# snap-research/3dgp

Hardware: AMD Instinct MI355X
Metric: generator-forward img/s @256^2, 64 steps (higher is better)
Workload: dtype f32; 1 GPU; BASELINE configs[2]: ImageNet 256x256, 64(+64) ray steps, cmax 512, c_dim 1000, tri-plane 512^2 x 96, full HIP path; batch_per_gpu=16, global_batch=16, img_resolution=256, num_ray_steps=64, depth_adaptor=False, parallelism=dp1 (batch-sharded, weights replicated)

## Files before the change

### 3dgp_amd/csrc/modconv.hip

```cpp
#include <type_traits>
#include "common.h"
#include <stdlib.h>

#ifndef TDGP_AB_NO_SCALAR_WV
#define TDGP_AB_NO_SCALAR_WV 0
#endif
#ifndef TDGP_AB_NO_PACKED_EPI
#define TDGP_AB_NO_PACKED_EPI 0
#endif
#ifndef TDGP_AB_FIR_SERIAL
#define TDGP_AB_FIR_SERIAL 0
#endif
#if TDGP_AB_NO_SCALAR_WV
#define TDGP_WAVE_INDEX(tid) ((tid) >> 6)
#else
#define TDGP_WAVE_INDEX(tid) __builtin_amdgcn_readfirstlane((tid) >> 6)
#endif

namespace {

typedef float f32x16 __attribute__((ext_vector_type(16)));

constexpr int KC3 = 4;

// ... 2741 lines not shown
                TDGP_LAUNCH("conv_mfma_kernel", conv3s_mfma_kernel, dim3((W >> 5) * cdiv(B * (H + 1), 8), cdiv(Cout, 64)), dim3(256), lds, s, q);
            } else if (g_conv_arith == 0 && TDGP_WINO4F_MAXCIN > 0 && out_layout == 0 && Cin <= TDGP_WINO4F_MAXCIN && (Cin & 15) == 0 && (Cout & 63) == 0 && wino4_txl(H, W) == 4 &&
                       wino4_shape_ok(B, Cin, Cout, H, W, k, up) && pi.wino4_floats > 0 && (int64_t)B * ((H * W) >> 9) * (Cout >> 6) >= 256 && !skip && ((uintptr_t)x & 15) == 0 &&
                       ((uintptr_t)y & 15) == 0 && (!noise || (((uintptr_t)noise & 15) == 0 && (noise_bstride & 3) == 0))) {
                float* vbuf = (float*)((char*)workspace + wl.wino_v);
                int* ticket = (int*)((char*)vbuf + ((wino4_v_bytes(wino4_sub_batch(B, Cin, Cout, H, W), Cin, H, W) + 255) / 256 * 256));
                const int cus = tdgp_cu_count(), nxcd = (cus % 8 == 0 && cus >= 64) ? 8 : 1, per = cus / nxcd, nsl = Cout >> 6;
                int rs = 1;
                while (rs * 2 <= nsl && (per % (rs * 2)) == 0 && (rs * 2) * 64 + per / (rs * 2) * 32 < rs * 64 + per / rs * 32) rs *= 2;
                Wino4fParams q;
                q.x = x; q.styles = styles; q.u = wp + pi.wp_floats + pi.wsq_floats + pi.wsplit_floats + pi.wbf_floats + pi.wino_floats; q.e = e;
                q.B = B; q.Cin = Cin; q.Cout = Cout; q.H = H; q.W = W; q.u_bytes = (uint32_t)(pi.wino4_floats * 4); q.x_bytes = c.x_bytes; q.st_bytes = c.st_bytes;
                q.nz_bytes = noise ? (uint32_t)(((noise_bstride ? (int64_t)(B - 1) * noise_bstride : 0) + (int64_t)H * W) * 4) : 0u;
                q.gxn = W / 64; q.gyn = H / 8; q.rs = rs; q.rt = per / rs; q.nxcd = nxcd; q.ticket = ticket;
                const size_t lds = (size_t)W4F_LDS_FLOATS * 4;
                TDGP_ONCE_PER_DEVICE((void)hipFuncSetAttribute((const void*)conv3_wino4f_kernel, hipFuncAttributeMaxDynamicSharedMemorySize, (int)lds););
                TDGP_CHECK(hipMemsetAsync(ticket, 0, 32, s) == hipSuccess, TDGP_ELAUNCH, "modconv2d: clearing the item counters failed");
                TDGP_LAUNCH("conv_wino4f_kernel", conv3_wino4f_kernel, dim3((unsigned)(nxcd * per)), dim3(512), lds, s, q);
            } else if (arith_wino4() && wino4_shape_ok(B, Cin, Cout, H, W, k, up, out_layout == 0) && pi.wino4_floats > 0 && (out_layout == 0 || out_layout == 2) && !skip && ((uintptr_t)x & 15) == 0 &&
                       ((uintptr_t)y & 15) == 0 && (!noise || (((uintptr_t)noise & 15) == 0 && (noise_bstride & 3) == 0))) {
                float* vbuf = (float*)((char*)workspace + wl.wino_v);
#ifndef TDGP_WINO4_PAIR
#define TDGP_WINO4_PAIR 1
#endif
                constexpr bool pairk = TDGP_WINO4_PAIR && W4_BM == 32;
                const int bpc = (W4_BM == 64 || pairk) ? 1 : 2;
                int ksl = (out_layout == 0 && !wino4_shape_ok(B, Cin, Cout, H, W, k, up)) ? wino4_ksplit_log2(B, Cin, Cout, H, W) : 0;
                const int64_t kslice = (int64_t)B * Cout * H * W;
                if ((kslice << ksl) > wl.partial_floats) ksl = 0;
                const int cus = tdgp_cu_count(), nxcd = (cus % 8 == 0 && cus >= 64) ? 8 : 1, per = cus / nxcd * bpc, nsl = cdiv(Cout, W4_BM) << ksl;
                int rs = 1;
                const int tpi = pairk ? 64 : 32;
                while (rs * 2 <= nsl && (per % (rs * 2)) == 0 && (rs * 2) * W4_BM + per / (rs * 2) * tpi < rs * W4_BM + per / rs * tpi) rs *= 2;
                const size_t lds = pairk ? (size_t)(8 * W4_UCH + 3 * W4_BM + 4) * 4 : (size_t)(2 * W4_STAGE + 2 * W4_BM + 4) * 4;
                TDGP_ONCE_PER_DEVICE((void)hipFuncSetAttribute((const void*)conv3_wino4_kernel<false, pairk>, hipFuncAttributeMaxDynamicSharedMemorySize, (int)lds); (void)hipFuncSetAttribute((const void*)conv3_wino4_kernel<true, pairk>, hipFuncAttributeMaxDynamicSharedMemorySize, (int)lds););
                const int bsub = ksl ? B : wino4_sub_batch(B, Cin, Cout, H, W);
                int* ticket = (int*)((char*)vbuf + ((wino4_v_bytes(wino4_sub_batch(B, Cin, Cout, H, W), Cin, H, W) + 255) / 256 * 256));
                for (int b0 = 0; b0 < B; b0 += bsub) {
                    const int bn = std::min(bsub, B - b0);
                    Wino4Params q;
                    q.v = vbuf; q.u = wp + pi.wp_floats + pi.wsq_floats + pi.wsplit_floats + pi.wbf_floats + pi.wino_floats; q.e = e;
                    q.e.y = y + (int64_t)b0 * Cout * H * W;
                    q.ups = out_layout == 2 ? 1 : 0;
                    if (e.dcoef) q.e.dcoef = e.dcoef + (int64_t)b0 * Cout;
                    if (e.noise) q.e.noise = e.noise + (int64_t)b0 * noise_bstride;
                    q.e.B = bn;
                    q.B = bn; q.Cin = Cin; q.Cout = Cout; q.CoutP = pi.CoutP; q.H = H; q.W = W;
                    q.v_bytes = (uint32_t)wino4_v_bytes(bn, Cin, H, W); q.u_bytes = (uint32_t)(pi.wino4_floats * 4);
                    q.txl = wino4_txl(H, W); q.gxn = W / (4 << q.txl); q.gyn = H / (128 >> q.txl);
                    q.rs = rs; q.rt = per / rs; q.nxcd = nxcd; q.ticket = ticket; q.ksl = ksl; q.partial = partial;
                    const int ntg = q.gxn * q.gyn * bn;
                    TDGP_LAUNCH("wino4_input_kernel", wino4_input_kernel, dim3((unsigned)(ntg * pi.nch4)), dim3(128), 0, s, x + (int64_t)b0 * Cin * H * W,
                                styles ? styles + (int64_t)b0 * Cin : nullptr, vbuf, bn, Cin, H, W, q.gxn, q.gyn, pi.nch4, q.txl, ticket);
                    if (q.ups) TDGP_LAUNCH("upconv_wino4_kernel", (conv3_wino4_kernel<true, pairk>), dim3((unsigned)(nxcd * per)), dim3(pairk ? 512 : W4_NW * 64), lds, s, q);
                    else TDGP_LAUNCH("conv_wino4_kernel", (conv3_wino4_kernel<false, pairk>), dim3((unsigned)(nxcd * per)), dim3(pairk ? 512 : W4_NW * 64), lds, s, q);
                    if (ksl) TDGP_LAUNCH("splitk_reduce_kernel", splitk_reduce_kernel, dim3((int)min((int64_t)2048, cdiv64(kslice, 256))), dim3(256), 0, s, partial, 1 << ksl, e);
                }
            } else if (k == 3 && (arith_wino4() || g_conv_arith == 3) && wino_ok(B, Cin, Cout, H, W) && out_layout == 0 && !skip && ((uintptr_t)x & 15) == 0 && ((uintptr_t)y & 7) == 0 &&
                       (!noise || (((uintptr_t)noise & 7) == 0 && (noise_bstride & 1) == 0))) {
                WinoParams q;
                q.x = x; q.u = wp + pi.wp_floats + pi.wsq_floats + pi.wsplit_floats + pi.wbf_floats; q.styles = styles; q.e = e;
                q.B = B; q.Cin = Cin; q.Cout = Cout; q.CoutP = pi.CoutP; q.H = H; q.W = W;
                q.x_bytes = c.x_bytes; q.u_bytes = (uint32_t)(pi.wino_floats * 4);
                const size_t lds = wino_lds_bytes(Cin);
                TDGP_ONCE_PER_DEVICE((void)hipFuncSetAttribute((const void*)conv3_wino_kernel, hipFuncAttributeMaxDynamicSharedMemorySize, 160 * 1024););
                if (TDGP_WINO_PERSIST) {
                    const int cus = tdgp_cu_count();
// ... 237 lines not shown
```

### 3dgp_amd/csrc/modconv_wino4.inc

```

typedef float f32x4 __attribute__((ext_vector_type(4)));

struct Wino4Params {
    const float* v; const float* u;
    EpiParams e;
    int B, Cin, Cout, CoutP, H, W;
    uint32_t v_bytes, u_bytes;
    int gxn, gyn;
    int txl;
    int rs, rt;
    int nxcd;
    int* ticket;
    int ups;
    int ksl;
    float* partial;
};

__device__ __forceinline__ void wino4_bt(const float (&d)[6], float (&t)[6]) {
    t[0] = fmaf_(1.5f, d[3] - d[1], fmaf_(-2.0f, d[2], d[0] + d[4]));
    t[1] = fmaf_(2.5f, d[3], fmaf_(0.5f, d[2], d[4] - d[1]));
    t[2] = fmaf_(-2.5f, d[2], fmaf_(0.5f, d[3], d[1] + d[4]));
    t[3] = fmaf_(2.0f, d[3] - d[1], d[4] - d[2]);
    t[4] = fmaf_(0.5f, d[1] - d[3], d[4] - d[2]);
    t[5] = fmaf_(1.5f, d[4] - d[2], fmaf_(-2.0f, d[3], d[1] + d[5]));
// ... 22 lines not shown
#pragma unroll
        for (int i = 0; i < 6; i++) col[i] = pr == 0 ? (w4_f2){acc[6 * i + j][0], acc[6 * i + j][1]} : (w4_f2){acc[6 * i + j][2], acc[6 * i + j][3]};
        w4_f2 y4[4];
        wino4_at2(col, y4);
#pragma unroll
        for (int a = 0; a < 4; a++) t[a][j] = y4[a];
    }
#pragma unroll
    for (int a = 0; a < 4; a++) wino4_at2(t[a], yy[a]);
}
template <int ACT>
__device__ __forceinline__ w4_f2 finish_pair(const EpiParams& e, w4_f2 v, w4_f2 d2, float nz, w4_f2 b2) {
    static_assert(ACT == 1 || ACT == 3, "packed output stage: linear / leaky ReLU without clamp");
    w4_f2 x = (v * d2 + (w4_f2){nz, nz}) + b2;
    if constexpr (ACT == 3) {
        const w4_f2 xa = x * (w4_f2){e.alpha, e.alpha};
        x = (w4_f2){__builtin_fmaxf(x.x, xa.x), __builtin_fmaxf(x.y, xa.y)};
    }
    return x * (w4_f2){e.gain, e.gain};
}

#ifndef TDGP_WINO4_MIN_C
#define TDGP_WINO4_MIN_C 64
#endif
#ifndef TDGP_WINO4_BM
#define TDGP_WINO4_BM 32
#endif
constexpr int W4_BM = TDGP_WINO4_BM, W4_NW = W4_BM / 8;
constexpr int W4_UCH = 9 * 4 * W4_BM * 4, W4_VCH = 9 * 4 * 32 * 4;
constexpr int W4_UP = W4_UCH / 256, W4_PAD = W4_BM == 64 ? 2 : 0;
constexpr int W4_NPW = (W4_UP + 18 + W4_PAD) / W4_NW;
constexpr int W4_STAGE = W4_UCH + W4_VCH + W4_PAD * 256;
static_assert((W4_UP + 18 + W4_PAD) % W4_NW == 0 && (W4_BM == 32 || W4_BM == 64), "wino4: piece count");

__global__ __launch_bounds__(256) void pack_wino4_kernel(const float* __restrict__ w, float* __restrict__ u, int Cout, int Cin, int nslice, int nch4) {
    const int64_t total = (int64_t)nslice * nch4 * W4_UCH;
    const double G[6][3] = {{1.0, 0.0, 0.0}, {1.0 / 3, 1.0 / 3, 1.0 / 3}, {-1.0 / 3, 1.0 / 3, -1.0 / 3}, {-16.0 / 15, -8.0 / 15, -4.0 / 15},
                            {1.0 / 15, -2.0 / 15, 4.0 / 15}, {0.0, 0.0, 1.0}};
    for (int64_t idx = blockIdx.x * (int64_t)blockDim.x + threadIdx.x; idx < total; idx += (int64_t)gridDim.x * blockDim.x) {
        const int e = (int)(idx & 3), cp = (int)(idx >> 2) % W4_BM, k = (int)((idx >> 2) / W4_BM) & 3;
        int64_t r = idx / (16 * W4_BM);
        const int xi4 = (int)(r % 9); r /= 9;
        const int ch = (int)(r % nch4), sl = (int)(r / nch4);
        const int o = sl * W4_BM + cp, c = ch * 4 + k, xi = 4 * xi4 + e, i = xi / 6, j = xi % 6;
        double v = 0.0;
        if (o < Cout && c < Cin) {
            const float* g = w + ((int64_t)o * Cin + c) * 9;
            for (int a = 0; a < 3; a++)
                for (int b = 0; b < 3; b++) v += G[i][a] * (double)g[a * 3 + b] * G[j][b];
        }
        u[idx] = (float)v;
    }
}

__global__ __launch_bounds__(128) void wino4_input_kernel(const float* __restrict__ x, const float* __restrict__ styles, float* __restrict__ v, int B, int Cin,
                                                          int H, int W, int gxn, int gyn, int nch4, int txl, int* __restrict__ ticket) {
    if (blockIdx.x == 0 && threadIdx.x < 8) ticket[threadIdx.x] = 0;
    const int k = threadIdx.x >> 5, t = threadIdx.x & 31, tx = t & ((1 << txl) - 1), ty = t >> txl;
    const int64_t blk = blockIdx.x;
    const int ch = (int)(blk % nch4);
    const int tg = (int)(blk / nch4);
    const int gx = tg % gxn, gy = (tg / gxn) % gyn, b = tg / (gxn * gyn);
    const int c = ch * 4 + k;
    const bool cok = c < Cin;
    const float s = (styles && cok) ? styles[b * Cin + c] : 1.0f;
    const int y0 = gy * (128 >> txl) + ty * 4 - 1, x0 = gx * (4 << txl) + tx * 4;
// ... 87 lines not shown
        const int q = wvx + 8 * i;
        dma(du, (uint32_t)__builtin_amdgcn_readfirstlane((int)(ust_lds + (uint32_t)q * 1024u)), lane16 + (uint32_t)q * 1024u, uo);
    };
    auto pairV = [&](int i, uint32_t vst_lds) {
        const int q = wvx + 8 * i;
        const bool second = i > 2 || (i == 2 && wvx >= 2);
        const int pc = second ? q - 18 : q;
        dma(dv, (uint32_t)__builtin_amdgcn_readfirstlane((int)(vst_lds + (second ? (uint32_t)(W4_VCH * 4) : 0u) + (uint32_t)pc * 1024u)), lane16 + (uint32_t)pc * 1024u, second ? vo1 : vo);
    };
    auto pair_offsets = [&](int cu, int cv) {
        uo = (uint32_t)__builtin_amdgcn_readfirstlane((int)(u_base + (uint32_t)cu * (W4_UCH * 4u)));
        vo = (uint32_t)__builtin_amdgcn_readfirstlane((int)(v_base + (uint32_t)cv * (W4_VCH * 4u)));
        vo1 = (uint32_t)__builtin_amdgcn_readfirstlane((int)(v_base1 + (uint32_t)cv * (W4_VCH * 4u)));
    };
    const uint32_t ldsU = lds0, ldsV = lds0 + 2u * (W4_UCH * 4u);
#ifndef TDGP_W4_EARLY_BARRIER
#define TDGP_W4_EARLY_BARRIER 0
#endif
    auto pair_first = [&](int nck) {
        pair_offsets(0, 0);
#pragma unroll
        for (int i = 0; i < 3; i++) if (i < 2 || wvx < 2) pairU(i, ldsU);
#pragma unroll
        for (int i = 0; i < 5; i++) if (i < 4 || wvx < 4) pairV(i, ldsV);
        pair_offsets(nck > 1 ? 1 : 0, nck > 1 ? 1 : 0);
        if (TDGP_W4_EARLY_BARRIER == 3) {
#pragma unroll
            for (int i = 0; i < 3; i++) if (i < 2 || wvx < 2) pairU(i, ldsU + (W4_UCH * 4u));
        }
#pragma unroll
        for (int i = 0; i < 5; i++) if (i < 4 || wvx < 4) pairV(i, ldsV + 2u * (W4_VCH * 4u));
    };

    int* const tk = (int*)(side + (PAIR ? 3 : 2) * W4_BM);
    const int per = p.rs * p.rt;
    auto from_ticket = [&](int t, int& sl, int& tg) {
        const int R = (t / per) * p.nxcd + xcd, j = t % per;
        if (R >= nrect) return -1;
        sl = (R % RS) * p.rs + j % p.rs;
        tg = (R / RS) * p.rt + j / p.rs;
        return (sl < nsl && tg < ntg) ? 1 : 0;
    };
    auto acquire = [&](int t_have, bool have_t, int& sl, int& tg) {
        for (;;) {
            if (tid == 0) tk[0] = have_t ? t_have : atomicAdd(p.ticket + xcd, 1);
            lds_barrier();
            const int t = tk[0];
            lds_barrier();
            const int st = from_ticket(t, sl, tg);
            if (st != 0) return st > 0;
            have_t = false;
        }
    };
    int sl = 0, tg = 0;
    bool have = acquire(0, false, sl, tg);
    auto set_bases = [&](int sl_, int tg_) {
        const uint32_t c0 = (uint32_t)(sl_ & ((1 << p.ksl) - 1)) * (uint32_t)nchk;
        u_base = ((uint32_t)(sl_ >> p.ksl) * (uint32_t)nch + c0) * (W4_UCH * 4u);
        v_base = ((uint32_t)(PAIR ? 2 * tg_ : tg_) * (uint32_t)nch + c0) * (W4_VCH * 4u);
        if (PAIR) v_base1 = ((uint32_t)min(2 * tg_ + 1, ntg1 - 1) * (uint32_t)nch + c0) * (W4_VCH * 4u);
    };
    if (have) {
        set_bases(sl, tg);
        if (PAIR) pair_first(nchk); else issue(0, 0);
    }
#ifndef TDGP_W4_TRACE
#define TDGP_W4_TRACE 0
#endif
    uint64_t tr_t[8] = {0, 0, 0, 0, 0, 0, 0, 0}, tr_last = 0;
    auto tr_mark = [&](int i) { if (TDGP_W4_TRACE) { const uint64_t n = __builtin_amdgcn_s_memtime(); tr_t[i] += n - tr_last; tr_last = n; } };
    if (TDGP_W4_TRACE) tr_last = __builtin_amdgcn_s_memtime();
    while (have) {
        const int tgw = PAIR ? min(2 * tg + hsel, ntg1 - 1) : tg;
        const bool tg_ok = !PAIR || 2 * tg + hsel < ntg1;
        const int m0 = (sl >> p.ksl) * W4_BM, gx = tgw % p.gxn, gy = (tgw / p.gxn) % p.gyn, b = tgw / (p.gxn * p.gyn);
        int t_next = 0;
        if (tid == 0) t_next = atomicAdd(p.ticket + xcd, 1);
        if (tid < (PAIR ? 3 : 2) * W4_BM) {
            const int o = m0 + (tid % W4_BM), hh = tid / W4_BM;
            float vv = hh == 0 ? 0.f : 1.f;
            if (o < p.Cout) {
                if (hh == 0) { if (p.e.bias) vv = p.e.bias[o]; }
                else if (p.e.dcoef) vv = p.e.dcoef[((PAIR ? min(2 * tg + hh - 1, ntg1 - 1) : tg) / (p.gxn * p.gyn)) * p.e.Cout + o];
            }
            side[tid] = vv;
        }
        f32x4 acc[36];
#pragma unroll
        for (int i = 0; i < 36; i++) acc[i] = (f32x4){0.f, 0.f, 0.f, 0.f};
        tr_mark(0);
        wait_loads();
        lds_barrier();
        tr_mark(1);
        if constexpr (PAIR) {
            int vs = 0;
            float4 fa[3], fb[3];
            auto frags_at = [&](const float* ust_, const float* vst_, int g, int q) {
                fa[q] = *(const float4*)(ust_ + g * (16 * W4_BM) + a_lane);
                fb[q] = *(const float4*)(vst_ + g * 512 + b_lane);
            };
            if (TDGP_W4_EARLY_BARRIER) {
                frags_at(smem, smem + 2 * W4_UCH + hsel * W4_VCH, 0, 0);
                frags_at(smem, smem + 2 * W4_UCH + hsel * W4_VCH, 1, 1);
            }
            for (int c = 0; c < nchk; c++) {
                const float* ust = smem + (c & 1) * W4_UCH;
                const float* vst = smem + 2 * W4_UCH + (vs * 2 + hsel) * W4_VCH;
                const uint32_t nus = ldsU + (uint32_t)((c + 1) & 1) * (W4_UCH * 4u);
                const int vs1 = vs == 2 ? 0 : vs + 1;
                const int vs2 = vs == 0 ? 2 : vs - 1;
                const float* ust1 = smem + ((c + 1) & 1) * W4_UCH;
                const float* vst1 = smem + 2 * W4_UCH + (vs1 * 2 + hsel) * W4_VCH;
                const uint32_t nvs = ldsV + (uint32_t)vs2 * (2u * W4_VCH * 4u);
                const uint32_t cus = ldsU + (uint32_t)(c & 1) * (W4_UCH * 4u);
                if (TDGP_W4_EARLY_BARRIER == 3) pair_offsets(c + 2 < nchk ? c + 2 : nchk - 1, c + 2 < nchk ? c + 2 : nchk - 1);
                else pair_offsets(c + 1 < nchk ? c + 1 : c, c + 2 < nchk ? c + 2 : nchk - 1);
                if (!TDGP_W4_EARLY_BARRIER) {
                    frags_at(ust, vst, 0, 0);
                    frags_at(ust, vst, 1, 1);
                }
#pragma unroll
                for (int g = 0; g < 9; g++) {
// ... 61 lines not shown
        }
        tr_mark(2);
        const int tt = tr * 16 + l15;
        const int oy = gy * (128 >> p.txl) + (tt >> p.txl) * 4, ox = gx * (4 << p.txl) + (tt & ((1 << p.txl) - 1)) * 4;
        constexpr bool NZ_LDS = PAIR && UPS;
        float* const nzw = smem + 2 * W4_UCH + 4 * W4_VCH + wvx * 1024;
        float4 nz[4];
#pragma unroll
        for (int a = 0; a < 4; a++) nz[a] = make_float4(0.f, 0.f, 0.f, 0.f);
        if (p.e.noise) {
            if constexpr (NZ_LDS) {
                const float* np = p.e.noise + b * p.e.noise_bstride + (int64_t)(2 * oy + 2 * kq) * (2 * p.W) + 2 * ox;
                nz[0] = *(const float4*)np; nz[1] = *(const float4*)(np + 4);
                nz[2] = *(const float4*)(np + 2 * p.W); nz[3] = *(const float4*)(np + 2 * p.W + 4);
            } else if constexpr (!UPS) {
                const float* np = p.e.noise + b * p.e.noise_bstride + (int64_t)oy * p.W + ox;
#pragma unroll
                for (int a = 0; a < 4; a++) nz[a] = *(const float4*)(np + (int64_t)a * p.W);
            }
        }
        int nsl_ = 0, ntg_ = 0;
        const bool more = acquire(t_next, true, nsl_, ntg_);
        tr_mark(3);
        if constexpr (NZ_LDS) {
            float* d = nzw + ((2 * kq) * 16 + l15) * 8;
            *(float4*)d = nz[0]; *(float4*)(d + 4) = nz[1];
            *(float4*)(d + 128) = nz[2]; *(float4*)(d + 132) = nz[3];
        } else if constexpr (!UPS) {
            asm volatile("" : "+v"(nz[0].x), "+v"(nz[0].w), "+v"(nz[1].x), "+v"(nz[1].w), "+v"(nz[2].x), "+v"(nz[2].w), "+v"(nz[3].x), "+v"(nz[3].w));
        }
        __builtin_amdgcn_sched_barrier(0);
        if (more) {
            set_bases(nsl_, ntg_);
            if (PAIR) pair_first(nchk); else issue(0, 0);
        }
        tr_mark(4);
        {
            auto up_noise = [&](int r, float4& n0, float4& n1) {
                n0 = make_float4(0.f, 0.f, 0.f, 0.f); n1 = n0;
                if constexpr (!NZ_LDS) { if (!p.e.noise) return; }
                if constexpr (NZ_LDS) {
                    const float* q = nzw + (r * 16 + l15) * 8;
                    n0 = *(const float4*)q; n1 = *(const float4*)(q + 4);
                } else {
                    const float* np = p.e.noise + b * p.e.noise_bstride + (int64_t)(2 * oy + r) * (2 * p.W) + 2 * ox;
                    n0 = *(const float4*)np; n1 = *(const float4*)(np + 4);
                }
            };
            auto write_outputs = [&](auto act_tag) {
                constexpr int ACT = decltype(act_tag)::value;
#pragma unroll
                for (int r = 0; r < 4; r++) {
                    const int chl = cg * 16 + kq * 4 + r, o = m0 + chl;
                    float t[4][6];
#pragma unroll
                    for (int j = 0; j < 6; j++) {
                        const float col[6] = {acc[j][r], acc[6 + j][r], acc[12 + j][r], acc[18 + j][r], acc[24 + j][r], acc[30 + j][r]};
                        float y4[4];
                        wino4_at(col, y4);
#pragma unroll
                        for (int a = 0; a < 4; a++) t[a][j] = y4[a];
                    }
                    if (o < p.Cout && tg_ok) {
                        const float dd = side[W4_BM * (1 + hsel) + chl], bs = side[chl];
                        float* yp = p.e.y + (((int64_t)b * p.Cout + o) * p.H + oy) * p.W + ox;
#pragma unroll
                        for (int a = 0; a < 4; a++) {
                            float y4[4];
                            wino4_at(t[a], y4);
                            *(float4*)(yp + (int64_t)a * p.W) = finish_act4<ACT>(p.e, make_float4(y4[0], y4[1], y4[2], y4[3]), dd, nz[a], bs);
                        }
                    }
                }
            };
            auto write_up = [&](auto act_tag) {
                constexpr int ACT = decltype(act_tag)::value;
                const int och = (m0 >> 2) + cg * 4 + kq, Co = p.Cout >> 2, H2 = 2 * p.H, W2 = 2 * p.W;
                if (och < Co && tg_ok) {
                    const int chl = cg * 16 + kq * 4;
                    const float dd = side[W4_BM * (1 + hsel) + chl], bs = side[chl];
                    float* yp = p.e.y + (((int64_t)b * Co + och) * H2 + 2 * oy) * W2 + 2 * ox;
#pragma unroll
                    for (int py = 0; py < 2; py++) {
                        float t[2][4][6];
#pragma unroll
                        for (int px = 0; px < 2; px++)
#pragma unroll
                            for (int j = 0; j < 6; j++) {
                                const int r = 2 * py + px;
                                const float col[6] = {acc[j][r], acc[6 + j][r], acc[12 + j][r], acc[18 + j][r], acc[24 + j][r], acc[30 + j][r]};
                                float y4[4];
                                wino4_at(col, y4);
#pragma unroll
                                for (int a = 0; a < 4; a++) t[px][a][j] = y4[a];
                            }
#pragma unroll
                        for (int a = 0; a < 4; a++) {
                            float e0[4], e1[4];
                            wino4_at(t[0][a], e0);
                            wino4_at(t[1][a], e1);
                            const int64_t ro = (int64_t)(2 * a + py) * W2;
                            float4 n0, n1;
                            up_noise(2 * a + py, n0, n1);
                            *(float4*)(yp + ro) = finish_act4<ACT>(p.e, make_float4(e0[0], e1[0], e0[1], e1[1]), dd, n0, bs);
                            *(float4*)(yp + ro + 4) = finish_act4<ACT>(p.e, make_float4(e0[2], e1[2], e0[3], e1[3]), dd, n1, bs);
                        }
                    }
                }
            };
            auto write_partial = [&]() {
                float* part = p.partial + (int64_t)(sl & ((1 << p.ksl) - 1)) * ((int64_t)p.B * p.Cout * p.H * p.W);
#pragma unroll
                for (int r = 0; r < 4; r++) {
                    const int o = m0 + cg * 16 + kq * 4 + r;
                    float t[4][6];
#pragma unroll
                    for (int j = 0; j < 6; j++) {
                        const float col[6] = {acc[j][r], acc[6 + j][r], acc[12 + j][r], acc[18 + j][r], acc[24 + j][r], acc[30 + j][r]};
                        float y4[4];
                        wino4_at(col, y4);
#pragma unroll
                        for (int a = 0; a < 4; a++) t[a][j] = y4[a];
                    }
                    if (o < p.Cout && tg_ok) {
                        float* yp = part + (((int64_t)b * p.Cout + o) * p.H + oy) * p.W + ox;
#pragma unroll
                        for (int a = 0; a < 4; a++) {
                            float y4[4];
                            wino4_at(t[a], y4);
                            *(float4*)(yp + (int64_t)a * p.W) = make_float4(y4[0], y4[1], y4[2], y4[3]);
                        }
                    }
                }
            };
            auto write_outputs_pk = [&](auto act_tag) {
                constexpr int ACT = decltype(act_tag)::value;
#pragma unroll
                for (int pr = 0; pr < 2; pr++) {
                    const int chl = cg * 16 + kq * 4 + 2 * pr, o = m0 + chl;
                    w4_f2 yy[4][4];
                    wino4_output_pair(acc, pr, yy);
                    if (tg_ok && o < p.Cout) {
                        const bool two = o + 1 < p.Cout;
                        const w4_f2 d2 = {side[W4_BM * (1 + hsel) + chl], side[W4_BM * (1 + hsel) + chl + 1]}, b2 = {side[chl], side[chl + 1]};
                        float* yp = p.e.y + (((int64_t)b * p.Cout + o) * p.H + oy) * p.W + ox;
                        const int64_t cs = (int64_t)p.H * p.W;
#pragma unroll
                        for (int a = 0; a < 4; a++) {
                            const float nq[4] = {nz[a].x, nz[a].y, nz[a].z, nz[a].w};
                            w4_f2 f[4];
#pragma unroll
                            for (int i = 0; i < 4; i++) f[i] = finish_pair<ACT>(p.e, yy[a][i], d2, nq[i], b2);
                            *(float4*)(yp + (int64_t)a * p.W) = make_float4(f[0].x, f[1].x, f[2].x, f[3].x);
                            if (two) *(float4*)(yp + cs + (int64_t)a * p.W) = make_float4(f[0].y, f[1].y, f[2].y, f[3].y);
                        }
                    }
                }
            };
            auto write_up_pk = [&](auto act_tag) {
                constexpr int ACT = decltype(act_tag)::value;
                const int och = (m0 >> 2) + cg * 4 + kq, Co = p.Cout >> 2, H2 = 2 * p.H, W2 = 2 * p.W;
                const int chl = cg * 16 + kq * 4;
                const float dd = side[W4_BM * (1 + hsel) + chl], bs = side[chl];
                const w4_f2 d2 = {dd, dd}, b2 = {bs, bs};
                float* yp = p.e.y + (((int64_t)b * Co + och) * H2 + 2 * oy) * W2 + 2 * ox;
#pragma unroll
                for (int py = 0; py < 2; py++) {
                    w4_f2 yy[4][4];
                    wino4_output_pair(acc, py, yy);
                    if (och < Co && tg_ok) {
#pragma unroll
                        for (int a = 0; a < 4; a++) {
                            const int64_t ro = (int64_t)(2 * a + py) * W2;
                            float4 n0, n1;
                            up_noise(2 * a + py, n0, n1);
                            auto fin = [&](w4_f2 v, float na, float nb) {
                                w4_f2 x = (v * d2 + (w4_f2){na, nb}) + b2;
                                if constexpr (ACT == 3) { const w4_f2 xa = x * (w4_f2){p.e.alpha, p.e.alpha}; x = (w4_f2){__builtin_fmaxf(x.x, xa.x), __builtin_fmaxf(x.y, xa.y)}; }
                                return x * (w4_f2){p.e.gain, p.e.gain};
                            };
                            const w4_f2 f0 = fin(yy[a][0], n0.x, n0.y), f1 = fin(yy[a][1], n0.z, n0.w), f2 = fin(yy[a][2], n1.x, n1.y), f3 = fin(yy[a][3], n1.z, n1.w);
                            *(float4*)(yp + ro) = make_float4(f0.x, f0.y, f1.x, f1.y);
                            *(float4*)(yp + ro + 4) = make_float4(f2.x, f2.y, f3.x, f3.y);
                        }
                    }
                }
            };
#ifndef TDGP_WINO4_PACKED_EPI
#define TDGP_WINO4_PACKED_EPI 1
#endif
            const int evar = epi_variant(p.e);
            if (!UPS && p.ksl > 0) write_partial();
            else
            if constexpr (UPS) {
                if (TDGP_WINO4_PACKED_EPI && evar == 3) write_up_pk(std::integral_constant<int, 3>{});
                else if (TDGP_WINO4_PACKED_EPI && evar == 1) write_up_pk(std::integral_constant<int, 1>{});
                else if (evar == 3) write_up(std::integral_constant<int, 3>{});
                else if (evar == 1) write_up(std::integral_constant<int, 1>{});
                else write_up(std::integral_constant<int, 0>{});
            } else {
                if (TDGP_WINO4_PACKED_EPI && evar == 3) write_outputs_pk(std::integral_constant<int, 3>{});
                else if (TDGP_WINO4_PACKED_EPI && evar == 1) write_outputs_pk(std::integral_constant<int, 1>{});
                else if (evar == 3) write_outputs(std::integral_constant<int, 3>{});
                else if (evar == 1) write_outputs(std::integral_constant<int, 1>{});
                else write_outputs(std::integral_constant<int, 0>{});
            }
            asm volatile("" :: "v"(nz[0].x), "v"(nz[0].w), "v"(nz[1].x), "v"(nz[1].w), "v"(nz[2].x), "v"(nz[2].w), "v"(nz[3].x), "v"(nz[3].w));
        }
        tr_mark(5);
        lds_barrier();
        tr_mark(6);
        if (TDGP_W4_TRACE) tr_t[7] += 1;
        have = more; sl = nsl_; tg = ntg_;
    }
    if (TDGP_W4_TRACE && tid == 0) {
        for (int i = 0; i < 8; i++) ((uint32_t*)p.e.y)[blockIdx.x * 8 + i] = (uint32_t)tr_t[i];
    }
}
```

### 3dgp_amd/isa_check.py

```python
import re


class IsaListingError(RuntimeError):
    """The assembly listing does not have the shape the checker parses (not a violation of the property it checks)."""


def _regs(tok):
    out = set()
    for m in re.finditer(r'v\[(\d+):(\d+)\]', tok):
        out.update(range(int(m.group(1)), int(m.group(2)) + 1))
    for m in re.finditer(r'(?<![\w\[:])v(\d+)\b', tok):
        out.add(int(m.group(1)))
    return out


def _code(lines):
    return [ln for ln in lines if ln.strip() and not ln.strip().startswith(';') and not ln.startswith('.')]


def check_kernel(body, fq):
    heads = [i for i, ln in enumerate(body) if 'Loop Header: Depth=1' in ln]
    if not heads:
        raise IsaListingError("no 'Loop Header: Depth=1' comment in the listing of triplane_walk2_kernel: this hipcc does not annotate loops "
                              '(asm-verbose off, or a different compiler) -- the check cannot locate the producer loop')
# ... 31 lines not shown
            if op.startswith('buffer_load_dwordx4') or op.startswith('global_load'):
                dst = _regs(ins.split(',')[0])
                if any(dst & d for d, _ in inflight):
                    bad.append(('load into a register that is still in flight', ins))
                if any(_regs(','.join(ins.split(',')[1:])) & d for d, _ in inflight):
                    bad.append(('address register is in flight', ins))
                nloads += lap == 0 and op.startswith('buffer_load')
                inflight.append((dst, ins))
                continue
            if op.startswith('s_'):
                continue
            touched = [t for d, t in inflight if _regs(ins) & d]
            if touched:
                bad.append((f'touches the destination of `{touched[0]}`', ins))
    if nloads == 0 and hand_waits == 0:
        return dict(loop_instructions=len(loop), tap_loads=0, hand_waits=0, compiler_vmcnt_waits=comp_waits, skipped='no hand-issued loads'), []
    if nloads != 6 * fq or hand_waits != 2:
        bad.append((f'expected {6 * fq} tap loads and 2 hand-written waits in the producer loop, found {nloads} / {hand_waits}', ''))
    return dict(loop_instructions=len(loop), tap_loads=nloads, hand_waits=hand_waits, compiler_vmcnt_waits=comp_waits), bad


def check_walk2_asm(asm_text):
    lines = asm_text.splitlines()
    out = {}
    for i, ln in enumerate(lines):
        m = re.match(r'^(_ZN\S*triplane_walk2_kernelILi(\d+)ELi(\d+)ELb([01])E\S*):', ln)
        if not m:
            continue
        end = next((j for j in range(i, len(lines)) if lines[j].strip().startswith('.amdhsa_kernel')), len(lines))
        out[m.group(1)] = check_kernel(lines[i:end], int(m.group(2)))
    return out


def check_wino4_kernel(body):
    code = [(i, ln.split(';')[0].strip()) for i, ln in enumerate(body)]
    code = [(i, c) for i, c in code if c and not c.startswith('.') or re.match(r'^\.LBB\d+_\d+:', c or '')]
    bad = []
    ins_only = [(i, c) for i, c in code if not c.endswith(':')]
    m0_writes = 0
    for k, (i, c) in enumerate(ins_only):
        if not re.search(r'\bm0\b', c):
            continue
        if not re.match(r'^s_mov_b32 m0, s\d+$', c):
            bad.append(('m0 is touched by an instruction other than the hand-written `s_mov_b32 m0, <sgpr>`', c))
            continue
        m0_writes += 1
        nxt = [x for _, x in ins_only[k + 1:k + 3]]
        if len(nxt) < 2 or nxt[0] != 's_nop 0' or not (nxt[1].startswith('buffer_load_dwordx4') and nxt[1].endswith(' lds')):
            bad.append(('`s_mov_b32 m0` is not followed by `s_nop 0` + an LDS-direct buffer load', c + ' | ' + ' | '.join(nxt)))
    waits = [k for k, (_, c) in enumerate(code) if re.match(r'^s_waitcnt vmcnt\(4\)$', c)]
    summary = dict(m0_writes=m0_writes, pair_loops=len(waits))
    k_loops = 0
    for w in waits:
        lab = next((code[k][1][:-1] for k in range(w, -1, -1) if code[k][1].endswith(':')), None)
        back = [k for k in range(w, len(code)) if re.match(r'^s_c?branch\w* ' + re.escape(lab or '?') + '$', code[k][1])]
        if lab is None or not back:
            continue
        k0 = next(k for k in range(w, -1, -1) if code[k][1] == lab + ':')
        loop = [c for _, c in code[k0:back[-1] + 1] if not c.endswith(':')]
        if not any(c.startswith('v_mfma') for c in loop):
            continue
        k_loops += 1
        vmem = [c for c in loop if re.match(r'^(buffer_|global_|flat_|scratch_)', c)]
        notlds = [c for c in vmem if not (c.startswith('buffer_load_dwordx4') and c.endswith(' lds'))]
        for c in notlds:
            bad.append(('a vector-memory instruction other than an LDS-direct load inside the K loop (the hand-counted vmcnt(4) does not know it)', c))
        if len(vmem) - len(notlds) != 8:
            bad.append((f'expected 8 LDS-direct issue sites (3 U + 5 V) in the K loop, found {len(vmem) - len(notlds)}', ''))
        descs = [re.search(r'(s\[\d+:\d+\])', c).group(1) for c in vmem if c not in notlds]
        if len(set(descs)) != 2 or descs != [descs[0]] * descs.count(descs[0]) + [descs[-1]] * descs.count(descs[-1]) or descs.count(descs[0]) != 3:
            bad.append(('the U loads (3 sites, one descriptor) must be issued before the V loads (5 sites, the other descriptor)', ' '.join(descs)))
        vwaits = [c for c in loop if c.startswith('s_waitcnt') and 'vmcnt' in c]
        if vwaits != ['s_waitcnt vmcnt(4)']:
            bad.append(('the K loop must hold exactly one vector-memory wait, the hand-written vmcnt(4)', ' | '.join(vwaits)))
        summary.update(loop_instructions=len(loop), lds_direct_sites=len(vmem) - len(notlds), mfma=sum(c.startswith('v_mfma') for c in loop))
    summary['pair_loops'] = k_loops
    return summary, bad


def check_wino4_asm(asm_text):
    lines = asm_text.splitlines()
    out = {}
    for i, ln in enumerate(lines):
        m = re.match(r'^(_ZN\S*conv3_wino4_kernelILb([01])ELb([01])E\S*):', ln)
        if not m:
            continue
        end = next((j for j in range(i, len(lines)) if lines[j].strip().startswith('.amdhsa_kernel')), len(lines))
        out[m.group(1)] = check_wino4_kernel(lines[i:end])
    return out


def check_wino4f_kernel(body):
    code = [(i, ln.split(';')[0].strip()) for i, ln in enumerate(body)]
    code = [c for _, c in code if c and (not c.startswith('.') or re.match(r'^\.LBB\d+_\d+:', c))]
    ins = [c for c in code if not c.endswith(':')]
    bad = []
    lds_direct = lambda c: re.match(r'^buffer_load_dword(x4)? ', c) and c.endswith(' lds')
    m0_writes = 0
    for k, c in enumerate(ins):
        if not re.search(r'\bm0\b', c):
            continue
        if not re.match(r'^s_mov_b32 m0, (s\d+|vcc_lo|vcc_hi|ttmp\d+)$', c):
            bad.append(('m0 is touched by an instruction other than the hand-written `s_mov_b32 m0, <sgpr>`', c))
            continue
        m0_writes += 1
        nxt = ins[k + 1:k + 3]
        if len(nxt) < 2 or nxt[0] != 's_nop 0' or not lds_direct(nxt[1]):
            bad.append(('`s_mov_b32 m0` is not followed by `s_nop 0` + an LDS-direct buffer load', c + ' | ' + ' | '.join(nxt)))
    for c in ins:
        if c.startswith('scratch_'):
            bad.append(('scratch access (a spill: its reload waits with vmcnt(0) for every LDS-direct load in flight)', c))
            break
    mf = [k for k, c in enumerate(code) if c.startswith('v_mfma')]
    if len(mf) != 144:
        raise IsaListingError(f'conv3_wino4f_kernel: expected 144 MFMAs (4 chunks x 36), found {len(mf)}')
    k0 = back = None
    for k in range(mf[0], -1, -1):
        if code[k].endswith(':'):
            bk = [j for j in range(mf[-1], len(code)) if re.match(r'^s_c?branch\w* ' + re.escape(code[k][:-1]) + '$', code[j])]
            if bk:
                k0, back = k, bk[0]
# ... 17 lines not shown
        for c2 in ins[k + 1:]:
            if c2 == 's_waitcnt vmcnt(0)':
                break
            if re.search(r'\b' + m.group(1) + r'\b', c2):
                bad.append((f'{m.group(1)}, the destination of a returning atomic, is touched before the next vmcnt(0)', c2))
                break
    item_back = next((k for k in range(len(code) - 1, back, -1) if re.match(r'^s_c?branch\w* \.LBB\d+_\d+$', code[k])), len(code) - 1)
    around = {code[k].split()[-1] for k in range(k0) if re.match(r'^s_c?branch\w* \.LBB\d+_\d+$', code[k])}
    tail, skip = [], False
    for c in code[back + 1:item_back]:
        if c.endswith(':'):
            skip = c[:-1] in around
            continue
        if not skip:
            tail.append(c)
    for k, c in enumerate(tail):
        if re.match(r'^(buffer_load|global_load|flat_load)', c) and not lds_direct(c):
            bad.append(('a vector-memory load of the compiler\'s behind the K loop (its wait would also wait for the next item\'s requests)', c))
        if c.startswith('s_waitcnt') and 'vmcnt' in c:
            prev = tail[max(0, k - 4):k]
            if not any(x.startswith('global_atomic_add') for x in prev):
                bad.append(('a vector-memory wait behind the K loop that does not belong to the ticket retry path', c))
    return dict(m0_writes=m0_writes, mfma=len(mf), loop_instructions=len(loop), lds_direct_sites=len(vmem), atomics=atomics, stores_behind_loop=sum(c.startswith('global_store') for c in tail)), bad


def check_wino4f_asm(asm_text):
    lines = asm_text.splitlines()
    out = {}
    for i, ln in enumerate(lines):
        m = re.match(r'^(_Z\S*conv3_wino4f_kernel\S*):', ln)
        if not m:
            continue
        end = next((j for j in range(i, len(lines)) if lines[j].strip().startswith('.amdhsa_kernel')), len(lines))
        out[m.group(1)] = check_wino4f_kernel(lines[i:end])
    return out


def check_torgb_kernel(body, mt):
    code, hand, in_asm = [], [], False
    for ln in body:
        t = ln.strip()
        if t.startswith(';;#ASMSTART'):
            in_asm = True
            continue
        if t.startswith(';;#ASMEND'):
            in_asm = False
            continue
        c = ln.split(';')[0].strip()
        if c and not c.startswith('.') and not c.endswith(':'):
            code.append(c)
            hand.append(in_asm)
    bad = []
    if any(c.startswith('scratch_') for c in code):
        bad.append(('scratch access in a ToRGB kernel with hand-counted tap waits', next(c for c in code if c.startswith('scratch_'))))
    hw = [k for k, c in enumerate(code) if hand[k] and re.match(r'^s_waitcnt vmcnt\(\d+\)$', c)]
    hl = [k for k, c in enumerate(code) if hand[k] and c.startswith('global_load_dwordx4')]
    ends = [n for n, k in enumerate(hw) if code[k] == 's_waitcnt vmcnt(0)']
    if not hw or not ends or ends[-1] != len(hw) - 1 or len(hl) != 4 * len(hw) or len(hw) % (4 * mt):
        bad.append((f'expected stages of hand-counted waits ending in vmcnt(0), 4 MT batches per tile and four tap loads per wait; found {len(hw)} waits, {len(hl)} loads', ''))
        return dict(batches=len(hw), tap_loads=len(hl), hand_waits=len(hw)), bad
    bounds = [0] + [n + 1 for n in ends]
    stages = len(ends)
    for st in range(stages):
        nb = bounds[st + 1] - bounds[st]
        w, ld_ = hw[bounds[st]:bounds[st + 1]], hl[4 * bounds[st]:4 * bounds[st + 1]]
        counts = [int(re.search(r'\((\d+)\)', code[k]).group(1)) for k in w]
        ahead = counts[0] // 4
# ... 47 lines not shown
```

Measured before the change: 729.9 img/s.

## Prefetch wino4 bias/dcoef side data via double-buffered LDS-direct loads

The persistent wino4 conv kernel used to load per-item bias and demodulation coefficients with ordinary global loads into shared memory at the start of each item. It also ended every item with a barrier. Those side values are now requested with LDS-direct buffer loads one item ahead, into a double-buffered side area, so the trailing barrier can be dropped. The ticket atomic becomes inline asm, and the accumulators are pinned with empty asm constraints to avoid spills. The ISA checker gains tests for scratch spills, atomic-destination hazards and stray vector-memory waits in the output stage. The risk is races on the side buffers, since the barrier is gone and correctness now rests on the parity scheme and the existing waits.

```diff
diff --git a/3dgp_amd/csrc/modconv.hip b/3dgp_amd/csrc/modconv.hip
--- a/3dgp_amd/csrc/modconv.hip
+++ b/3dgp_amd/csrc/modconv.hip
@@ -2797,7 +2797,7 @@
                 int rs = 1;
                 const int tpi = pairk ? 64 : 32;
                 while (rs * 2 <= nsl && (per % (rs * 2)) == 0 && (rs * 2) * W4_BM + per / (rs * 2) * tpi < rs * W4_BM + per / rs * tpi) rs *= 2;
-                const size_t lds = pairk ? (size_t)(8 * W4_UCH + 3 * W4_BM + 4) * 4 : (size_t)(2 * W4_STAGE + 2 * W4_BM + 4) * 4;
+                const size_t lds = (size_t)((pairk ? 8 * W4_UCH : 2 * W4_STAGE) + W4_SIDE + 4) * 4;
                 TDGP_ONCE_PER_DEVICE((void)hipFuncSetAttribute((const void*)conv3_wino4_kernel<false, pairk>, hipFuncAttributeMaxDynamicSharedMemorySize, (int)lds); (void)hipFuncSetAttribute((const void*)conv3_wino4_kernel<true, pairk>, hipFuncAttributeMaxDynamicSharedMemorySize, (int)lds););
                 const int bsub = ksl ? B : wino4_sub_batch(B, Cin, Cout, H, W);
                 int* ticket = (int*)((char*)vbuf + ((wino4_v_bytes(wino4_sub_batch(B, Cin, Cout, H, W), Cin, H, W) + 255) / 256 * 256));
diff --git a/3dgp_amd/csrc/modconv_wino4.inc b/3dgp_amd/csrc/modconv_wino4.inc
--- a/3dgp_amd/csrc/modconv_wino4.inc
+++ b/3dgp_amd/csrc/modconv_wino4.inc
@@ -78,6 +78,8 @@
 constexpr int W4_NPW = (W4_UP + 18 + W4_PAD) / W4_NW;
 constexpr int W4_STAGE = W4_UCH + W4_VCH + W4_PAD * 256;
 static_assert((W4_UP + 18 + W4_PAD) % W4_NW == 0 && (W4_BM == 32 || W4_BM == 64), "wino4: piece count");
+constexpr int W4_SIDE_SET = 3 * 64;
+constexpr int W4_SIDE = 2 * W4_SIDE_SET;
 
 __global__ __launch_bounds__(256) void pack_wino4_kernel(const float* __restrict__ w, float* __restrict__ u, int Cout, int Cin, int nslice, int nch4) {
     const int64_t total = (int64_t)nslice * nch4 * W4_UCH;
@@ -231,7 +233,7 @@
         for (int i = 0; i < 5; i++) if (i < 4 || wvx < 4) pairV(i, ldsV + 2u * (W4_VCH * 4u));
     };
 
-    int* const tk = (int*)(side + (PAIR ? 3 : 2) * W4_BM);
+    int* const tk = (int*)(side + W4_SIDE);
     const int per = p.rs * p.rt;
     auto from_ticket = [&](int t, int& sl, int& tg) {
         const int R = (t / per) * p.nxcd + xcd, j = t % per;
@@ -251,7 +253,20 @@
             have_t = false;
         }
     };
-    int sl = 0, tg = 0;
+    if (!p.e.dcoef)
+        for (int i = tid; i < W4_SIDE; i += (int)blockDim.x) side[i] = 1.0f;
+    auto request_side = [&](int sl_, int tg_, int par_) {
+        const int sw = (PAIR ? 7 : W4_NW - 1) - wvx;
+        if (sw > (PAIR ? 2 : 1) || (sw > 0 && !p.e.dcoef)) return;
+        const int mo = (sl_ >> p.ksl) * W4_BM;
+        const int bs_ = (PAIR ? min(2 * tg_ + (sw == 2 ? 1 : 0), ntg1 - 1) : tg_) / (p.gxn * p.gyn);
+        const w4_u32x4 dd = sw == 0 ? desc(p.e.bias ? (const void*)p.e.bias : (const void*)p.u, p.e.bias ? (uint32_t)p.Cout * 4u : 0u)
+                                    : desc(p.e.dcoef, (uint32_t)(p.e.B * p.e.Cout) * 4u);
+        const uint32_t dst = (uint32_t)__builtin_amdgcn_readfirstlane((int)(TDGP_LDS_BASE(side) + (uint32_t)(par_ * W4_SIDE_SET + sw * 64) * 4u));
+        const uint32_t vo_ = (uint32_t)((sw == 0 ? mo : bs_ * p.e.Cout + mo) + l) * 4u;
+        asm volatile("s_mov_b32 m0, %0\n\ts_nop 0\n\tbuffer_load_dword %1, %2, %3 offen lds" :: "s"(dst), "v"(vo_), "s"(dd), "s"(0u) : "memory");
+    };
+    int sl = 0, tg = 0, par = 0;
     bool have = acquire(0, false, sl, tg);
     auto set_bases = [&](int sl_, int tg_) {
         const uint32_t c0 = (uint32_t)(sl_ & ((1 << p.ksl) - 1)) * (uint32_t)nchk;
@@ -261,6 +276,7 @@
     };
     if (have) {
         set_bases(sl, tg);
+        request_side(sl, tg, 0);
         if (PAIR) pair_first(nchk); else issue(0, 0);
     }
 #ifndef TDGP_W4_TRACE
@@ -273,20 +289,16 @@
         const int tgw = PAIR ? min(2 * tg + hsel, ntg1 - 1) : tg;
         const bool tg_ok = !PAIR || 2 * tg + hsel < ntg1;
         const int m0 = (sl >> p.ksl) * W4_BM, gx = tgw % p.gxn, gy = (tgw / p.gxn) % p.gyn, b = tgw / (p.gxn * p.gyn);
-        int t_next = 0;
-        if (tid == 0) t_next = atomicAdd(p.ticket + xcd, 1);
-        if (tid < (PAIR ? 3 : 2) * W4_BM) {
-            const int o = m0 + (tid % W4_BM), hh = tid / W4_BM;
-            float vv = hh == 0 ? 0.f : 1.f;
-            if (o < p.Cout) {
-                if (hh == 0) { if (p.e.bias) vv = p.e.bias[o]; }
-                else if (p.e.dcoef) vv = p.e.dcoef[((PAIR ? min(2 * tg + hh - 1, ntg1 - 1) : tg) / (p.gxn * p.gyn)) * p.e.Cout + o];
-            }
-            side[tid] = vv;
-        }
+        int t_next = 1;
+        if (tid == 0) asm volatile("global_atomic_add %0, %1, %0, %2 sc0" : "+v"(t_next) : "v"(xcd * 4), "s"(p.ticket) : "memory");
+        const float* const sd = side + par * W4_SIDE_SET;
         f32x4 acc[36];
 #pragma unroll
         for (int i = 0; i < 36; i++) acc[i] = (f32x4){0.f, 0.f, 0.f, 0.f};
+#pragma unroll
+        for (int i = 0; i < 36; i += 12)
+            asm volatile("" : "+v"(acc[i]), "+v"(acc[i + 1]), "+v"(acc[i + 2]), "+v"(acc[i + 3]), "+v"(acc[i + 4]), "+v"(acc[i + 5]), "+v"(acc[i + 6]), "+v"(acc[i + 7]), "+v"(acc[i + 8]),
+                         "+v"(acc[i + 9]), "+v"(acc[i + 10]), "+v"(acc[i + 11]));
         tr_mark(0);
         wait_loads();
         lds_barrier();
@@ -414,6 +426,7 @@
         __builtin_amdgcn_sched_barrier(0);
         if (more) {
             set_bases(nsl_, ntg_);
+            request_side(nsl_, ntg_, par ^ 1);
             if (PAIR) pair_first(nchk); else issue(0, 0);
         }
         tr_mark(4);
@@ -444,7 +457,7 @@
                         for (int a = 0; a < 4; a++) t[a][j] = y4[a];
                     }
                     if (o < p.Cout && tg_ok) {
-                        const float dd = side[W4_BM * (1 + hsel) + chl], bs = side[chl];
+                        const float dd = sd[64 * (1 + hsel) + chl], bs = sd[chl];
                         float* yp = p.e.y + (((int64_t)b * p.Cout + o) * p.H + oy) * p.W + ox;
 #pragma unroll
                         for (int a = 0; a < 4; a++) {
@@ -460,7 +473,7 @@
                 const int och = (m0 >> 2) + cg * 4 + kq, Co = p.Cout >> 2, H2 = 2 * p.H, W2 = 2 * p.W;
                 if (och < Co && tg_ok) {
                     const int chl = cg * 16 + kq * 4;
-                    const float dd = side[W4_BM * (1 + hsel) + chl], bs = side[chl];
+                    const float dd = sd[64 * (1 + hsel) + chl], bs = sd[chl];
                     float* yp = p.e.y + (((int64_t)b * Co + och) * H2 + 2 * oy) * W2 + 2 * ox;
 #pragma unroll
                     for (int py = 0; py < 2; py++) {
@@ -524,7 +537,7 @@
                     wino4_output_pair(acc, pr, yy);
                     if (tg_ok && o < p.Cout) {
                         const bool two = o + 1 < p.Cout;
-                        const w4_f2 d2 = {side[W4_BM * (1 + hsel) + chl], side[W4_BM * (1 + hsel) + chl + 1]}, b2 = {side[chl], side[chl + 1]};
+                        const w4_f2 d2 = {sd[64 * (1 + hsel) + chl], sd[64 * (1 + hsel) + chl + 1]}, b2 = {sd[chl], sd[chl + 1]};
                         float* yp = p.e.y + (((int64_t)b * p.Cout + o) * p.H + oy) * p.W + ox;
                         const int64_t cs = (int64_t)p.H * p.W;
 #pragma unroll
@@ -543,7 +556,7 @@
                 constexpr int ACT = decltype(act_tag)::value;
                 const int och = (m0 >> 2) + cg * 4 + kq, Co = p.Cout >> 2, H2 = 2 * p.H, W2 = 2 * p.W;
                 const int chl = cg * 16 + kq * 4;
-                const float dd = side[W4_BM * (1 + hsel) + chl], bs = side[chl];
+                const float dd = sd[64 * (1 + hsel) + chl], bs = sd[chl];
                 const w4_f2 d2 = {dd, dd}, b2 = {bs, bs};
                 float* yp = p.e.y + (((int64_t)b * Co + och) * H2 + 2 * oy) * W2 + 2 * ox;
 #pragma unroll
@@ -590,10 +603,9 @@
             asm volatile("" :: "v"(nz[0].x), "v"(nz[0].w), "v"(nz[1].x), "v"(nz[1].w), "v"(nz[2].x), "v"(nz[2].w), "v"(nz[3].x), "v"(nz[3].w));
         }
         tr_mark(5);
-        lds_barrier();
         tr_mark(6);
         if (TDGP_W4_TRACE) tr_t[7] += 1;
-        have = more; sl = nsl_; tg = ntg_;
+        have = more; sl = nsl_; tg = ntg_; par ^= 1;
     }
     if (TDGP_W4_TRACE && tid == 0) {
         for (int i = 0; i < 8; i++) ((uint32_t*)p.e.y)[blockIdx.x * 8 + i] = (uint32_t)tr_t[i];
diff --git a/3dgp_amd/isa_check.py b/3dgp_amd/isa_check.py
--- a/3dgp_amd/isa_check.py
+++ b/3dgp_amd/isa_check.py
@@ -87,7 +87,17 @@
     return out
 
 
-def check_wino4_kernel(body):
+def _private_segment_bytes(lines, name):
+    for i, ln in enumerate(lines):
+        if ln.split() == ['.amdhsa_kernel', name]:
+            for l2 in lines[i:i + 80]:
+                m = re.match(r'^\s*\.amdhsa_private_segment_fixed_size\s+(\d+)', l2)
+                if m:
+                    return int(m.group(1))
+    return None
+
+
+def check_wino4_kernel(body, pair=False, private_bytes=0):
     code = [(i, ln.split(';')[0].strip()) for i, ln in enumerate(body)]
     code = [(i, c) for i, c in code if c and not c.startswith('.') or re.match(r'^\.LBB\d+_\d+:', c or '')]
     bad = []
@@ -101,11 +111,29 @@
             continue
         m0_writes += 1
         nxt = [x for _, x in ins_only[k + 1:k + 3]]
-        if len(nxt) < 2 or nxt[0] != 's_nop 0' or not (nxt[1].startswith('buffer_load_dwordx4') and nxt[1].endswith(' lds')):
+        if len(nxt) < 2 or nxt[0] != 's_nop 0' or not (re.match(r'^buffer_load_dword(x4)? ', nxt[1]) and nxt[1].endswith(' lds')):
             bad.append(('`s_mov_b32 m0` is not followed by `s_nop 0` + an LDS-direct buffer load', c + ' | ' + ' | '.join(nxt)))
+    for _, c in ins_only:
+        if c.startswith('scratch_'):
+            bad.append(('scratch access (a spill: its reload waits with vmcnt(0) for every LDS-direct load in flight)', c))
+            break
+    if private_bytes:
+        bad.append((f'private segment of {private_bytes} bytes (expected 0: no spill)', ''))
+    atomics = 0
+    for k, (_, c) in enumerate(ins_only):
+        m = re.match(r'^global_atomic_add (v\d+),', c)
+        if not m:
+            continue
+        atomics += 1
+        for _, c2 in ins_only[k + 1:]:
+            if c2 == 's_waitcnt vmcnt(0)':
+                break
+            if re.search(r'\b' + m.group(1) + r'\b', c2):
+                bad.append((f'{m.group(1)}, the destination of a returning atomic, is touched before the next vmcnt(0)', c2))
+                break
     waits = [k for k, (_, c) in enumerate(code) if re.match(r'^s_waitcnt vmcnt\(4\)$', c)]
-    summary = dict(m0_writes=m0_writes, pair_loops=len(waits))
-    k_loops = 0
+    summary = dict(m0_writes=m0_writes, pair_loops=len(waits), atomics=atomics)
+    k_loops, k_end = 0, None
     for w in waits:
         lab = next((code[k][1][:-1] for k in range(w, -1, -1) if code[k][1].endswith(':')), None)
         back = [k for k in range(w, len(code)) if re.match(r'^s_c?branch\w* ' + re.escape(lab or '?') + '$', code[k][1])]
@@ -116,6 +144,7 @@
         if not any(c.startswith('v_mfma') for c in loop):
             continue
         k_loops += 1
+        k_end = back[-1]
         vmem = [c for c in loop if re.match(r'^(buffer_|global_|flat_|scratch_)', c)]
         notlds = [c for c in vmem if not (c.startswith('buffer_load_dwordx4') and c.endswith(' lds'))]
         for c in notlds:
@@ -130,6 +159,21 @@
             bad.append(('the K loop must hold exactly one vector-memory wait, the hand-written vmcnt(4)', ' | '.join(vwaits)))
         summary.update(loop_instructions=len(loop), lds_direct_sites=len(vmem) - len(notlds), mfma=sum(c.startswith('v_mfma') for c in loop))
     summary['pair_loops'] = k_loops
+    if pair and k_loops == 0:
+        raise IsaListingError('conv3_wino4_kernel (PAIR): no K loop recognised (a loop with MFMAs that ends in the hand-written `s_waitcnt vmcnt(4)`)')
+    if k_end is not None:
+        item_back = next((k for k in range(len(code) - 1, k_end, -1) if re.match(r'^s_c?branch\w* \.LBB\d+_\d+$', code[k][1])), len(code) - 1)
+        tail = [c for _, c in code[k_end + 1:item_back] if not c.endswith(':')]
+        first = next((k for k, c in enumerate(tail) if c.startswith('s_mov_b32 m0')), None)
+        if first is None:
+            bad.append(('no LDS-direct request (the next item\'s first chunks) behind the K loop', ''))
+        else:
+            for k, c in enumerate(tail[first:], first):
+                if re.match(r'^(buffer_load|global_load|flat_load|scratch_load)', c) and not c.endswith(' lds'):
+                    bad.append(('a vector-memory load of the compiler\'s in the output stage (its wait would also wait for the next item\'s requests)', c))
+                if c.startswith('s_waitcnt') and 'vmcnt' in c and not any(x.startswith('global_atomic_add') for x in tail[max(0, k - 4):k]):
+                    bad.append(('a vector-memory wait in the output stage (it also waits for the next item\'s requests)', c))
+            summary.update(stores_behind_requests=sum(c.startswith('global_store') for c in tail[first:]))
     return summary, bad
 
 
@@ -141,7 +185,7 @@
         if not m:
             continue
         end = next((j for j in range(i, len(lines)) if lines[j].strip().startswith('.amdhsa_kernel')), len(lines))
-        out[m.group(1)] = check_wino4_kernel(lines[i:end])
+        out[m.group(1)] = check_wino4_kernel(lines[i:end], pair=m.group(3) == '1', private_bytes=_private_segment_bytes(lines[end:end + 80], m.group(1)) or 0)
     return out
 
 
@@ -225,7 +269,11 @@
         if not m:
             continue
         end = next((j for j in range(i, len(lines)) if lines[j].strip().startswith('.amdhsa_kernel')), len(lines))
-        out[m.group(1)] = check_wino4f_kernel(lines[i:end])
+        summary, bad = check_wino4f_kernel(lines[i:end])
+        priv = _private_segment_bytes(lines[end:end + 80], m.group(1))
+        if priv:
+            bad.append((f'private segment of {priv} bytes (expected 0: no spill)', ''))
+        out[m.group(1)] = (summary, bad)
     return out
 
 
```

New measurement: 729.4 img/s. About the same (-0.1%).
